# leggedrobotics/art_planner

Hardware: AMD Instinct MI355X
Metric: validated states/sec on 400x400@0.04m map (sample + validity check) (higher is better)
Workload: dtype f32; 1 GPU; C2: lazy_prm_star_min_update front end, 400x400@0.04m Perlin terrain (seed 1234) + 12 obstacles, YAML robot, batch sampler + validity checker; map=400x400@0.04, lanes=1

## Files before the change

art_planner_amd/csrc/artp_capi.hip:

```cpp
#include "../../include/artp_c.h"

#include <hip/hip_runtime.h>
#include <hipcub/hipcub.hpp>

#include <cmath>
#include <cstdio>
#include <atomic>
#include <chrono>
#include <cstdlib>
#include <cstring>
#include <mutex>
#include <string>
#include <array>
#include <vector>

#include "pipeline.h"
#include "cost_kernels.h"

using namespace artp;

#define ARTP_FEW_STATES 16
#define ARTP_SVC_MAX_STATES 2
#define FEW_EDGE_S1 0
#define FEW_EDGE_S2 (ARTP_FEW_EDGES * 7 * sizeof(double))
// ... 12 lines not shown
  RobotDev robot{};
  MapGeom geom{};
  bool have_geom = false;
  std::atomic<uint64_t> map_version{0};
  FieldDev field[2]{};
  float* field_data[2] = {nullptr, nullptr};
  size_t field_elems[2] = {0, 0};
  bool have_field[2] = {false, false};
  void* rect_stage_host = nullptr;
  void* rect_stage_dev = nullptr;
  size_t rect_stage_cap = 0;
  hipEvent_t rect_stage_done = nullptr;
  hipEvent_t map_written = nullptr;
  hipEvent_t lane_mark[4] = {nullptr, nullptr, nullptr, nullptr};
  uint64_t map_write_seq = 0;
  uint64_t map_seen[4] = {0, 0, 0, 0};
  SamplerDev sampler{};
  float* sampler_buf = nullptr;
  float* sampler_pack = nullptr;
  int sampler_rows = 0, sampler_cols = 0;
  bool have_sampler = false;
  double z_low = 0.0, z_high = 0.0;
  bool have_z = false;
  int fc_mfma_wanted = 1;
  artp_cost_query_fn ext_cost_fn = nullptr;
  void* ext_cost_user = nullptr;
  bool few_edges = true;
  bool edge_two_pass = true;
  int edge_coarse_stride = ARTP_COARSE_STRIDE;
  float* table_buf[2] = {nullptr, nullptr};
  unsigned char* flag_buf[2] = {nullptr, nullptr};
  unsigned* stride_buf[2] = {nullptr, nullptr};
  unsigned char* partner_buf[2] = {nullptr, nullptr};
  unsigned* partner_cnt[2] = {nullptr, nullptr};
  int* d_diff = nullptr;
  int partner_R_built[2] = {-1, -1};
  int layer_has_nonfinite[2] = {1, 1};
  float4* tri_raw_buf[2] = {nullptr, nullptr};
  size_t table_elems[2] = {0, 0};
  TablesDev tables[2]{};
  ScratchCaps caps_full{0, 0, 0, 0};
  ScratchCaps caps_scan{0, 0, 0, 0};
  ScratchCaps caps_feet{0, 0, 0, 0};
  ScratchCaps caps_feet_wave{0, 0, 0, 0};
  ScratchCaps caps_foot_full{0, 0, 0, 0};
  int n_cus = 256;
  double* pin_states = nullptr;
  volatile uint8_t* pin_labels = nullptr;
  double* pin_states_dev = nullptr;
  uint8_t* pin_labels_dev = nullptr;
  bool poll_labels = true;
  bool svc_enabled = false, svc_launched = false;
  hipStream_t svc_stream = nullptr;
  hipEvent_t svc_after_map = nullptr;
  SvcMailbox* svc = nullptr;
  SvcMailbox* svc_dev = nullptr;
  uint32_t svc_seq = 0;
  uint64_t svc_map_version = 0;
  uint64_t svc_launches = 0, svc_requests = 0;
  bool pool_launched = false;
  hipStream_t pool_stream = nullptr;
  hipEvent_t pool_after_map = nullptr;
  EdgeMailbox* pool_mb = nullptr;
  int pool_bar = -1;
  PoolResponse* pool_resp = nullptr;
  PoolResponse* pool_resp_dev = nullptr;
  PoolCtl* pool_ctl = nullptr;
  uint64_t pool_shadow[5][7] = {};
  unsigned pool_wgs = ARTP_POOL_WGS;
  uint32_t pool_seq = 0;
  uint64_t pool_map_version = 0;
  uint64_t pool_launches = 0, pool_requests = 0;
  char* pin_edges_in = nullptr;
  char* pin_edges_in_dev = nullptr;
  char* pin_edges = nullptr;
  char* pin_edges_dev = nullptr;
  FewEdgeSync* d_few_sync = nullptr;
  int* d_error = nullptr;
  unsigned long long* d_count = nullptr;
  void* tmp[8] = {nullptr, nullptr, nullptr, nullptr, nullptr, nullptr, nullptr, nullptr};
  size_t tmp_cap[8] = {0, 0, 0, 0, 0, 0, 0, 0};
  void* cub_tmp = nullptr;
  size_t cub_cap = 0;
  struct lane_state {
    bool init = false;
    hipStream_t own_stream = nullptr, stream = nullptr;
    unsigned long long* d_count = nullptr;
    int* d_error = nullptr;
    void* tmp[8] = {nullptr, nullptr, nullptr, nullptr, nullptr, nullptr, nullptr, nullptr};
    size_t tmp_cap[8] = {0, 0, 0, 0, 0, 0, 0, 0};
    void* cub_tmp = nullptr;
    size_t cub_cap = 0;
  };
  lane_state lanes[ARTP_MAX_LANES];
  int cur_lane = 0;
  bool have_weights = false;
  int cost_net = 0;
  half8* d_convw[5] = {nullptr, nullptr, nullptr, nullptr, nullptr};
  float* d_convb[5] = {nullptr, nullptr, nullptr, nullptr, nullptr};
  float* d_c12 = nullptr;
  unsigned char* d_c12m = nullptr;
  int conv12_mfma = 1;
  half8* d_convw_chunk[3] = {nullptr, nullptr, nullptr};
  half8* d_convw_p32 = nullptr;
  float* d_fc = nullptr;
  char* d_fc_mfma = nullptr;
  int feet_dense = 0;
  double r3_extent_override = 0.0;
  int fc_mfma = 1;
  int fc_selfcheck = -1;
  float fc_selfcheck_err = 0.f;
  half_t* d_act[2] = {nullptr, nullptr};
  size_t act_cap = 0;
  half_t* d_feat = nullptr;
  size_t feat_cap = 0;
  float* d_map_f32 = nullptr;
  size_t map_cap = 0;
  CostMapGeom cost_geom{};
  int feat_h = 0, feat_w = 0;
  bool have_features = false;
  bool cost_fill_holes = false;
  bool cost_fill_telea = false;
  std::string last_error;
  std::string arch;
  std::recursive_mutex mu;
};

namespace {

#define HIP_TRY(ctx, expr)                                                        \
  do {                                                                            \
    hipError_t _e = (expr);                                                       \
    if (_e != hipSuccess) {                                                       \
      (ctx)->last_error = std::string(#expr) + ": " + hipGetErrorString(_e);      \
      return ARTP_ERR_HIP;                                                        \
    }                                                                             \
  } while (0)

int ensure_tmp(artp_ctx* c, int slot, size_t bytes) {
  if (c->tmp_cap[slot] >= bytes) return ARTP_OK;
  if (c->tmp[slot]) HIP_TRY(c, hipFree(c->tmp[slot]));
  c->tmp[slot] = nullptr;
  c->tmp_cap[slot] = 0;
  const size_t want = bytes + bytes / 4 + 256;
  HIP_TRY(c, hipMalloc(&c->tmp[slot], want));
  c->tmp_cap[slot] = want;
  return ARTP_OK;
}

void park_lane(artp_ctx* c) {
  artp_ctx::lane_state& l = c->lanes[c->cur_lane];
  l.init = true;
  l.own_stream = c->own_stream;
  l.stream = c->stream;
  l.d_count = c->d_count;
  l.d_error = c->d_error;
  l.cub_tmp = c->cub_tmp;
  l.cub_cap = c->cub_cap;
  for (int k = 0; k < 8; ++k) {
    l.tmp[k] = c->tmp[k];
    l.tmp_cap[k] = c->tmp_cap[k];
  }
}

void unpark_lane(artp_ctx* c, int lane) {
  const artp_ctx::lane_state& l = c->lanes[lane];
  c->own_stream = l.own_stream;
  c->stream = l.stream;
  c->d_count = l.d_count;
  c->d_error = l.d_error;
  c->cub_tmp = l.cub_tmp;
  c->cub_cap = l.cub_cap;
  for (int k = 0; k < 8; ++k) {
    c->tmp[k] = l.tmp[k];
    c->tmp_cap[k] = l.tmp_cap[k];
  }
  c->cur_lane = lane;
}

int order_after_other_lanes(artp_ctx* c) {
  for (int l = 0; l < ARTP_MAX_LANES; ++l) {
    if (l == c->cur_lane || !c->lanes[l].init) continue;
    if (!c->lane_mark[l]) HIP_TRY(c, hipEventCreateWithFlags(&c->lane_mark[l], hipEventDisableTiming));
    HIP_TRY(c, hipEventRecord(c->lane_mark[l], c->lanes[l].stream));
    HIP_TRY(c, hipStreamWaitEvent(c->stream, c->lane_mark[l], 0));
  }
  return ARTP_OK;
}

int publish_map_write(artp_ctx* c) {
  if (!c->map_written) HIP_TRY(c, hipEventCreateWithFlags(&c->map_written, hipEventDisableTiming));
  HIP_TRY(c, hipEventRecord(c->map_written, c->stream));
  c->map_seen[c->cur_lane] = ++c->map_write_seq;
  return ARTP_OK;
}

int lane_sees_map(artp_ctx* c) {
  if (c->map_seen[c->cur_lane] != c->map_write_seq && c->map_written) {
    HIP_TRY(c, hipStreamWaitEvent(c->stream, c->map_written, 0));
    c->map_seen[c->cur_lane] = c->map_write_seq;
  }
  return ARTP_OK;
}

void fill_robot(artp_ctx* c) {
  const artp_params& p = c->params;
  RobotDev& r = c->robot;
  r.torso[0] = (float)p.torso_length;
  r.torso[1] = (float)p.torso_width;
  r.torso[2] = (float)p.torso_height;
  r.foot[0] = (float)p.reach_x;
  r.foot[1] = (float)p.reach_y;
  r.foot[2] = (float)p.reach_z;
  r.torso_off[0] = (float)p.torso_off_x;
  r.torso_off[1] = (float)p.torso_off_y;
  r.torso_off[2] = (float)(p.torso_off_z - p.feet_off_z);
  r.feet_off_x = (float)p.feet_off_x;
  r.feet_off_y = (float)p.feet_off_y;
  r.unknown_space_untraversable = p.unknown_space_untraversable;
  r.reach_z = p.reach_z;
  r.max_pitch_pert = p.max_pitch_pert;
  r.max_roll_pert = p.max_roll_pert;
}

void r_from_2_axes(float* R, float ax, float ay, float az, float bx, float by, float bz) {
  float l = sqrtf(ax * ax + ay * ay + az * az);
  if (l <= 0.0f) return;
  l = 1.0f / l;
  ax *= l; ay *= l; az *= l;
  const float k = ax * bx + ay * by + az * bz;
  bx -= k * ax; by -= k * ay; bz -= k * az;
  l = sqrtf(bx * bx + by * by + bz * bz);
  if (l <= 0.0f) return;
  l = 1.0f / l;
  bx *= l; by *= l; bz *= l;
  R[0] = ax; R[4] = ay; R[8] = az;
  R[1] = bx; R[5] = by; R[9] = bz;
  R[2] = -by * az + ay * bz;
  R[6] = -bz * ax + az * bx;
  R[10] = -bx * ay + ax * by;
  R[3] = R[7] = R[11] = 0.0f;
}

int size_scratch(artp_ctx* c) {
  const artp_params& p = c->params;
  const double d_torso = std::sqrt(p.torso_length * p.torso_length + p.torso_width * p.torso_width +
                                   p.torso_height * p.torso_height);
  const double d_foot = std::sqrt(p.reach_x * p.reach_x + p.reach_y * p.reach_y + p.reach_z * p.reach_z);
  double diag = d_torso > d_foot ? d_torso : d_foot;
  double spacing = 1e30;
  int max_n = 2;
  for (int s = 0; s < 2; ++s) {
    if (!c->have_field[s]) continue;
    spacing = std::fmin(spacing, (double)std::fmin(c->field[s].sample_w, c->field[s].sample_d));
    max_n = std::max(max_n, std::max(c->field[s].nW, c->field[s].nD));
  }
  if (spacing > 1e29) return ARTP_OK;
  int maxdim = (int)std::ceil(diag / spacing) + 4;
  if (maxdim > max_n) maxdim = max_n;
  if (maxdim < 4) maxdim = 4;
  long verts = (long)maxdim * maxdim;
  long tris = 2L * (maxdim - 1) * (maxdim - 1);
  if (tris > 4096) tris = 4096;
  verts = (verts + 3) & ~3L;
  tris = (tris + 7) & ~7L;
  long tab = 64;
  while (tab < 2 * tris && tab < 4096) tab <<= 1;
  if (maxdim > 64) {
    c->last_error = "box window wider than 64 samples: not supported by the packed triangle ids";
    return ARTP_ERR_CAPACITY;
  }
  c->caps_full = ScratchCaps{64 * 36, (int)verts, (int)tris, (int)tab};
  c->caps_scan = ScratchCaps{64 * 36, (int)verts, (int)(tris < 1024 ? tris : 1024), 0};
  {
    int fdim = (int)std::ceil(d_foot / spacing) + 4;
    if (fdim > max_n) fdim = max_n;
    if (fdim < 4) fdim = 4;
    long fv = ((long)fdim * fdim + 3) & ~3L;
    long ft = (2L * (fdim - 1) * (fdim - 1) + 7) & ~7L;
    if (ft > 1024) ft = 1024;
    c->caps_feet = ScratchCaps{32 * 36, (int)fv, (int)ft, 0};
    c->caps_feet_wave = ScratchCaps{64 * 36, (int)fv, (int)ft, 0};
    long ftf = (2L * (fdim - 1) * (fdim - 1) + 7) & ~7L;
    if (ftf > 4096) ftf = 4096;
    long ftab = 64;
    while (ftab < 2 * ftf && ftab < 4096) ftab <<= 1;
    c->caps_foot_full = ScratchCaps{64 * 36, (int)fv, (int)ftf, (int)ftab};
  }
  if (scratch_bytes_per_wave(c->caps_full) > 160 * 1024 ||
      scratch_bytes_per_wave(c->caps_scan) * ARTP_WAVES_PER_BLOCK > 160 * 1024 ||
      scratch_bytes_per_wave(c->caps_full) + 4 * scratch_bytes_per_wave(c->caps_foot_full) > 160 * 1024) {
    c->last_error = "box too large for the LDS window tile";
    return ARTP_ERR_CAPACITY;
  }
  return ARTP_OK;
}

size_t lds_full(const artp_ctx* c) { return scratch_bytes_per_wave(c->caps_full); }
size_t lds_scan(const artp_ctx* c) { return scratch_bytes_per_wave(c->caps_scan) * ARTP_WAVES_PER_BLOCK; }
size_t lds_feet(const artp_ctx* c) { return scratch_bytes_per_wave(c->caps_feet) * 4 * ARTP_WAVES_PER_BLOCK; }
size_t lds_feet_wave(const artp_ctx* c) { return scratch_bytes_per_wave(c->caps_feet_wave) * ARTP_WAVES_PER_BLOCK; }
size_t lds_few(const artp_ctx* c) {
  return scratch_bytes_per_wave(c->caps_full) + 4 * scratch_bytes_per_wave(c->caps_foot_full);
}

int set_kernel_lds(artp_ctx* c) {
  HIP_TRY(c, hipFuncSetAttribute(reinterpret_cast<const void*>(check_boxes_kernel<1>),
                                 hipFuncAttributeMaxDynamicSharedMemorySize, (int)lds_full(c)));
  HIP_TRY(c, hipFuncSetAttribute(reinterpret_cast<const void*>(validate_states_kernel<1>),
                                 hipFuncAttributeMaxDynamicSharedMemorySize, (int)lds_full(c)));
  HIP_TRY(c, hipFuncSetAttribute(reinterpret_cast<const void*>(plane_stage_kernel<1>),
                                 hipFuncAttributeMaxDynamicSharedMemorySize, (int)lds_full(c)));
  HIP_TRY(c, hipFuncSetAttribute(reinterpret_cast<const void*>(validate_few_kernel),
                                 hipFuncAttributeMaxDynamicSharedMemorySize, (int)lds_few(c)));
  HIP_TRY(c, hipFuncSetAttribute(reinterpret_cast<const void*>(check_motions_few_kernel),
                                 hipFuncAttributeMaxDynamicSharedMemorySize, (int)lds_few(c)));
  HIP_TRY(c, hipFuncSetAttribute(reinterpret_cast<const void*>(resolve_boxes_kernel<ARTP_WAVES_PER_BLOCK, 64, 3>),
                                 hipFuncAttributeMaxDynamicSharedMemorySize, (int)lds_scan(c)));
  HIP_TRY(c, hipFuncSetAttribute(reinterpret_cast<const void*>(resolve_boxes_kernel<ARTP_WAVES_PER_BLOCK, 16, 1>),
                                 hipFuncAttributeMaxDynamicSharedMemorySize, (int)lds_feet(c)));
  HIP_TRY(c, hipFuncSetAttribute(reinterpret_cast<const void*>(resolve_boxes_kernel<ARTP_WAVES_PER_BLOCK, 64, 2>),
                                 hipFuncAttributeMaxDynamicSharedMemorySize, (int)lds_feet_wave(c)));
  return ARTP_OK;
}

int grid_full(const artp_ctx* c, size_t tasks) {
  size_t per_cu = (160 * 1024) / (lds_full(c) ? lds_full(c) : 1);
  if (per_cu > 16) per_cu = 16;
  if (per_cu < 1) per_cu = 1;
  size_t g = (size_t)c->n_cus * per_cu;
  if (tasks && tasks < g) g = tasks;
  return (int)(g ? g : 1);
}
int grid_scan(const artp_ctx* c, size_t lds) {
  size_t per_cu = (160 * 1024) / (lds ? lds : 1);
  if (per_cu > 8) per_cu = 8;
  if (per_cu < 1) per_cu = 1;
  return (int)((size_t)c->n_cus * per_cu);
}

unsigned grid_sub(const artp_ctx* c, int per_cu) {
  const unsigned g = (unsigned)c->n_cus * (unsigned)per_cu;
  return (g + ARTP_NSUB - 1) / ARTP_NSUB * ARTP_NSUB;
}

int partner_radius(const artp_ctx* c, int slot) {
  const FieldDev& f = c->field[slot];
  const float* side = slot == 1 ? c->robot.foot : c->robot.torso;
  const double diag = std::sqrt((double)side[0] * side[0] + (double)side[1] * side[1] + (double)side[2] * side[2]);
  const int R = (int)std::ceil(diag / std::fmin((double)f.sample_w, (double)f.sample_d)) + 3;
  return R > 63 ? -1 : R;
}

static void partner_rect_extent(const FieldDev& f, const PartnerRects& pr, int margin, int* max_cells, int* max_rows) {
  *max_cells = *max_rows = 1;
  for (int k = 0; k < pr.n; ++k) {
    const int nx = std::min(pr.x1[k] + margin, f.nW - 1) - std::max(pr.x0[k] - margin, 0) + 1;
    const int nz = std::min(pr.z1[k] + margin, f.nD - 1) - std::max(pr.z0[k] - margin, 0) + 1;
    *max_cells = std::max(*max_cells, nx * nz);
    *max_rows = std::max(*max_rows, pr.z1[k] - pr.z0[k] + 1);
  }
}

int build_partner_table_full(artp_ctx* c, int slot) {
  FieldDev& f = c->field[slot];
// ... 68 lines not shown
  FieldDev& f = c->field[slot];
  const int R = partner_radius(c, slot);
  int cells0, cellsR, rows;
  partner_rect_extent(f, pr, 0, &cells0, &rows);
  partner_rect_extent(f, pr, R, &cellsR, &rows);
  hipLaunchKernelGGL(tri_raw_rects_kernel, dim3((cells0 + 255) / 256, pr.n), dim3(256), 0, c->stream, f, pr,
                     c->tri_raw_buf[slot], c->partner_cnt[slot]);
  hipLaunchKernelGGL(partner_count_kernel<true>, dim3((cellsR + 255) / 256, rows, pr.n), dim3(256), 0, c->stream, f, R,
                     (const float4*)c->tri_raw_buf[slot], c->partner_cnt[slot], pr, 1);
  hipLaunchKernelGGL(partner_count_kernel<false>, dim3((cells0 + 255) / 256, 2 * R + 1, pr.n), dim3(256), 0, c->stream, f, R,
                     (const float4*)c->tri_raw_buf[slot], c->partner_cnt[slot], pr, 1);
  hipLaunchKernelGGL(partner_flags_from_counts_kernel, dim3((cellsR + 255) / 256, pr.n), dim3(256), 0, c->stream, f.nW, f.nD,
                     pr, R, (const unsigned*)c->partner_cnt[slot], c->partner_buf[slot]);
  HIP_TRY(c, hipGetLastError());
  c->partner_R_built[slot] = R;
  f.partner_flags = c->partner_buf[slot];
  f.partner_R = R;
  return ARTP_OK;
}

int build_tables(artp_ctx* c, int slot, const PartnerRects* pr = nullptr) {
  const FieldDev& f = c->field[slot];
  const size_t elems = (size_t)f.nW * f.nD;
  if (c->table_elems[slot] < elems) {
    if (c->table_buf[slot]) HIP_TRY(c, hipFree(c->table_buf[slot]));
    if (c->flag_buf[slot]) HIP_TRY(c, hipFree(c->flag_buf[slot]));
    if (c->stride_buf[slot]) HIP_TRY(c, hipFree(c->stride_buf[slot]));
    c->stride_buf[slot] = nullptr;
    if (c->partner_buf[slot]) HIP_TRY(c, hipFree(c->partner_buf[slot]));
    if (c->partner_cnt[slot]) HIP_TRY(c, hipFree(c->partner_cnt[slot]));
    c->partner_cnt[slot] = nullptr;
    HIP_TRY(c, hipMalloc(reinterpret_cast<void**>(&c->partner_cnt[slot]), elems * sizeof(unsigned)));
    if (c->tri_raw_buf[slot]) HIP_TRY(c, hipFree(c->tri_raw_buf[slot]));
    c->tri_raw_buf[slot] = nullptr;
    HIP_TRY(c, hipMalloc(reinterpret_cast<void**>(&c->tri_raw_buf[slot]), elems * sizeof(float4)));
    c->table_buf[slot] = nullptr;
    c->flag_buf[slot] = nullptr;
    c->partner_buf[slot] = nullptr;
    HIP_TRY(c, hipMalloc(reinterpret_cast<void**>(&c->partner_buf[slot]), (elems + 3) / 4 * 4));
    c->partner_R_built[slot] = -1;
    HIP_TRY(c, hipMalloc(reinterpret_cast<void**>(&c->table_buf[slot]), 12 * elems * sizeof(float)));
    HIP_TRY(c, hipMalloc(reinterpret_cast<void**>(&c->flag_buf[slot]), 6 * elems));
    HIP_TRY(c, hipMalloc(reinterpret_cast<void**>(&c->stride_buf[slot]), (elems / 2 + 3 * (f.nW + f.nD) + 16) * sizeof(unsigned)));
    c->table_elems[slot] = elems;
  }
  float2* mm[6];
  unsigned char* fl[6];
  for (int l = 0; l < 6; ++l) {
    mm[l] = reinterpret_cast<float2*>(c->table_buf[slot]) + (size_t)l * elems;
    fl[l] = reinterpret_cast<unsigned char*>(c->flag_buf[slot]) + (size_t)l * elems;
  }
  const int n = (int)elems;
  hipLaunchKernelGGL(table_level0_kernel, dim3((n + 255) / 256), dim3(256), 0, c->stream, f.data, n, mm[0], fl[0]);
  for (int l = 1; l < 6; ++l)
    hipLaunchKernelGGL(table_level_up_kernel, dim3((n + 255) / 256), dim3(256), 0, c->stream,
                       (const float2*)mm[l - 1], (const unsigned char*)fl[l - 1], f.nW, f.nD, 1 << (l - 1), mm[l],
                       fl[l]);
  HIP_TRY(c, hipGetLastError());
  TablesDev& t = c->tables[slot];
  t.mm = mm[2];
  t.fl = fl[2];
  t.stride = (unsigned)elems;
  t.has_nan = f.has_nan;
  t.has_nonfinite = c->layer_has_nonfinite[slot];
  {
    unsigned off[ARTP_STRIDE_LEVELS + 1] = {0};
    for (int l = 0; l < ARTP_STRIDE_LEVELS; ++l) {
      const int s = 2 << l;
      off[l + 1] = off[l] + (unsigned)(((f.nW + s - 1) / s) * ((f.nD + s - 1) / s));
    }
    t.st = c->stride_buf[slot];
    t.st_off1 = off[1];
    t.st_off2 = off[2];
    hipLaunchKernelGGL(stride_tables_kernel, dim3((off[3] + 255) / 256), dim3(256), 0, c->stream, t.mm, t.fl, t.stride,
                       f.nW, f.nD, off[1], off[2], off[3], c->stride_buf[slot]);
    HIP_TRY(c, hipGetLastError());
  }
  const int rc_partner = pr ? partner_update_end(c, slot, *pr) : build_partner_table_full(c, slot);
  if (rc_partner != ARTP_OK) return rc_partner;
  t.valid = 1;
  return ARTP_OK;
}

int ensure_recs(artp_ctx* c, size_t n) { return ensure_tmp(c, 7, n * sizeof(PoseRec)); }

int launch_validate_pipeline(artp_ctx* c, const double* se3, size_t n, uint8_t* valid, bool recs_ready = false) {
  if (n >= (1ull << 32)) {
    c->last_error = "batch too large (state index is 32 bit)";
    return ARTP_ERR_INVALID_ARG;
  }
  int rc = ensure_recs(c, n);
  if (rc) return rc;
  PoseRec* recs = static_cast<PoseRec*>(c->tmp[7]);
  if (!recs_ready)
    hipLaunchKernelGGL(pose_rec_kernel, dim3((unsigned)((n + 255) / 256)), dim3(256), 0, c->stream, c->field[0], se3, n,
                       recs);
  const size_t per_block_states = 64 * ARTP_CLASSIFY_SUB;
  const size_t n_blocks = (n + per_block_states - 1) / per_block_states;
  const size_t seg_t = ((n_blocks + ARTP_NSUB - 1) / ARTP_NSUB) * per_block_states;
  rc = ensure_tmp(c, 4, 5 * ARTP_NSUB * seg_t * sizeof(PendingBox));
  if (rc) return rc;
  const size_t ctr_bytes = 128 + (size_t)2 * ARTP_NSUB * 128;
  rc = ensure_tmp(c, 5, ctr_bytes + ((5 + 4 + 4) * n + 5 * (size_t)ARTP_NSUB * seg_t) * sizeof(unsigned) + 64);
  if (rc) return rc;
  PipelineQueues q;
  q.q1 = static_cast<PendingBox*>(c->tmp[4]);
  q.counters = static_cast<unsigned long long*>(c->tmp[5]);
  q.sub = q.counters + 16;
  q.seg_t = seg_t;
  q.q2 = reinterpret_cast<unsigned*>(static_cast<char*>(c->tmp[5]) + ctr_bytes);
  q.q3 = q.q2 + 5 * n;
  q.q5 = q.q3 + 4 * n;
  q.q4 = q.q5 + 4 * n;
  q.q6 = q.q4 + 4 * (size_t)ARTP_NSUB * seg_t;
  q.feet_base = (unsigned long long)ARTP_NSUB * seg_t;
  HIP_TRY(c, hipMemsetAsync(q.counters, 0, ctr_bytes, c->stream));
  const size_t per_block = 64 * ARTP_CLASSIFY_SUB;
  hipLaunchKernelGGL(classify_states_kernel, dim3((unsigned)((n + per_block - 1) / per_block)),
                     dim3(ARTP_CLASSIFY_THREADS), 0, c->stream,
                     c->field[0], c->field[1], c->tables[0], c->tables[1], c->geom, c->robot, (const PoseRec*)recs, n,
                     valid, q);
#ifdef ARTP_VARIANTS
  if (c->feet_dense)
    hipLaunchKernelGGL(feet_stream2_kernel<ARTP_STREAM_WAVES>, dim3(grid_sub(c, ARTP_FEET_WAVES_PER_SIMD)), dim3(64 * ARTP_STREAM_WAVES), 0,
                       c->stream, c->field[1], c->robot, q, valid);
  else
#endif
    hipLaunchKernelGGL(feet_stream_kernel<ARTP_STREAM_WAVES>, dim3(grid_sub(c, ARTP_FEET_WAVES_PER_SIMD)), dim3(64 * ARTP_STREAM_WAVES), 0,
                       c->stream, c->field[1], c->robot, q, valid);
  hipLaunchKernelGGL(feet_lane_kernel, dim3((unsigned)c->n_cus * 8), dim3(ARTP_LANE_THREADS), 0, c->stream,
                     c->field[1], c->robot, q, valid);
  {
    const ScratchCaps caps_stream{0, 0, 0, 0};
    const size_t lds_stream = 0;
    hipLaunchKernelGGL((resolve_boxes_kernel<ARTP_WAVES_PER_BLOCK, 64, 0>), dim3(grid_sub(c, ARTP_TORSO_WGS_PER_CU)),
                       dim3(64 * ARTP_WAVES_PER_BLOCK), lds_stream, c->stream, c->field[0], c->robot, q, valid,
                       caps_stream, c->d_error, c->tables[0].valid ? c->tables[0].mm : (const float2*)nullptr);
  }
  hipLaunchKernelGGL((resolve_boxes_kernel<ARTP_WAVES_PER_BLOCK, 64, 3>), dim3(grid_scan(c, lds_scan(c))),
                     dim3(64 * ARTP_WAVES_PER_BLOCK), lds_scan(c), c->stream, c->field[0], c->robot, q, valid,
                     c->caps_scan, c->d_error);
  hipLaunchKernelGGL((resolve_boxes_kernel<ARTP_WAVES_PER_BLOCK, 16, 1>), dim3(grid_scan(c, lds_feet(c))),
                     dim3(64 * ARTP_WAVES_PER_BLOCK), lds_feet(c), c->stream, c->field[1], c->robot, q, valid,
                     c->caps_feet, c->d_error);
  hipLaunchKernelGGL((resolve_boxes_kernel<ARTP_WAVES_PER_BLOCK, 64, 2>), dim3(grid_scan(c, lds_feet_wave(c))),
                     dim3(64 * ARTP_WAVES_PER_BLOCK), lds_feet_wave(c), c->stream, c->field[1], c->robot, q, valid,
                     c->caps_feet_wave, c->d_error);
  hipLaunchKernelGGL(plane_stage_kernel<1>, dim3(grid_full(c, 0)), dim3(64), lds_full(c), c->stream,
                     c->field[0], c->field[1], c->robot, q, valid, c->caps_full, c->d_error);
  HIP_TRY(c, hipGetLastError());
  return ARTP_OK;
}

int check_error_flag(artp_ctx* c) {
  int flag = 0;
  HIP_TRY(c, hipMemcpyAsync(&flag, c->d_error, sizeof(int), hipMemcpyDeviceToHost, c->stream));
  HIP_TRY(c, hipStreamSynchronize(c->stream));
  if (flag) {
    HIP_TRY(c, hipMemsetAsync(c->d_error, 0, sizeof(int), c->stream));
    c->last_error = "a box window exceeded the LDS tile capacity";
    return ARTP_ERR_CAPACITY;
  }
  return ARTP_OK;
}

}

extern "C" {

void artp_params_defaults(artp_params* p) {
  p->torso_length = 1.05; p->torso_width = 0.55; p->torso_height = 0.2;
  p->torso_off_x = 0.0; p->torso_off_y = 0.0; p->torso_off_z = 0.0;
  p->feet_off_x = 0.362; p->feet_off_y = 0.225; p->feet_off_z = -0.525;
  p->reach_x = 0.25; p->reach_y = 0.1; p->reach_z = 0.15;
  p->unknown_space_untraversable = 1;
  p->max_pitch_pert = 10.0 / 180 * M_PI;
  p->max_roll_pert = 3.33 / 180 * M_PI;
  p->sample_from_distribution = 1;
}

void artp_params_yaml(artp_params* p) {
  p->torso_length = 1.31; p->torso_width = 0.65; p->torso_height = 0.3;
  p->torso_off_x = 0.0; p->torso_off_y = 0.0; p->torso_off_z = 0.04;
  p->feet_off_x = 0.51; p->feet_off_y = 0.2; p->feet_off_z = -0.475;
  p->reach_x = 0.2; p->reach_y = 0.2; p->reach_z = 0.2;
  p->unknown_space_untraversable = 1;
  p->max_pitch_pert = 10 * M_PI / 180;
  p->max_roll_pert = 3.33 * M_PI / 180;
  p->sample_from_distribution = 1;
}

const char* artp_status_string(int s) {
  switch (s) {
    case ARTP_OK: return "ok";
    case ARTP_ERR_INVALID_ARG: return "invalid argument";
    case ARTP_ERR_NO_DEVICE: return "no usable HIP device (this library has no CPU fallback)";
    case ARTP_ERR_HIP: return "HIP runtime error";
    case ARTP_ERR_NO_MAP: return "required layer not uploaded";
    case ARTP_ERR_CAPACITY: return "box window exceeds the LDS tile capacity";
    case ARTP_ERR_NO_WEIGHTS: return "motion-cost weights not loaded";
    case ARTP_ERR_TIMEOUT: return "timed out waiting for a device group";
    case ARTP_ERR_COMM: return "RCCL unavailable or a communicator call failed";
    case ARTP_ERR_COST_FUNC: return "Motion cost call failed";
    default: return "unknown status";
  }
}

const char* artp_last_error(const artp_ctx* ctx) { return ctx ? ctx->last_error.c_str() : ""; }
const char* artp_device_arch(const artp_ctx* ctx) { return ctx ? ctx->arch.c_str() : ""; }

static void pool_stop(artp_ctx* c);
static void svc_stop(artp_ctx* c) {
  if (!c->svc || !c->svc_launched) return;
  c->svc->n_quit = 0x100u;
  std::atomic_thread_fence(std::memory_order_seq_cst);
  const auto t0 = std::chrono::steady_clock::now();
  while (c->svc->running && std::chrono::steady_clock::now() - t0 < std::chrono::milliseconds(200))
    ;
  (void)hipStreamSynchronize(c->svc_stream);
  c->svc_launched = false;
}

static int svc_start(artp_ctx* c) {
  if (!c->svc) {
    void *p = nullptr, *pd = nullptr;
    HIP_TRY(c, hipHostMalloc(&p, sizeof(SvcMailbox), hipHostMallocMapped));
    HIP_TRY(c, hipHostGetDevicePointer(&pd, p, 0));
    std::memset(p, 0, sizeof(SvcMailbox));
    c->svc = static_cast<SvcMailbox*>(p);
    c->svc_dev = static_cast<SvcMailbox*>(pd);
    HIP_TRY(c, hipStreamCreateWithFlags(&c->svc_stream, hipStreamNonBlocking));
    HIP_TRY(c, hipEventCreateWithFlags(&c->svc_after_map, hipEventDisableTiming));
    HIP_TRY(c, hipFuncSetAttribute(reinterpret_cast<const void*>(validate_service_kernel),
// ... 1435 lines not shown
  if (!c || (n && (!s1 || !s2 || !valid))) return ARTP_ERR_INVALID_ARG;
  if (n == 0) return ARTP_OK;
  std::lock_guard<std::recursive_mutex> lock(c->mu);
  HIP_TRY(c, hipSetDevice(c->device));
  double few_max = 0.0;
  if (n <= ARTP_FEW_EDGES && c->few_edges && c->have_field[0] && c->have_field[1] && (mode != 0 || c->have_z) &&
      few_edges_task_estimate(c, mode, s1, s2, n, &few_max) <= 65536.0) {
    if (c->svc_enabled && n <= ARTP_POOL_MAX_EDGES && few_max * n <= 8.0 * c->pool_wgs && pool_available(c))
      return run_edges_pool(c, mode, s1, s2, n, valid, aux_out, last_t, last_state);
    return run_edges_few(c, mode, true, s1, s2, n, valid, aux_out, last_t, last_state, few_max);
  }
  int rc = ensure_tmp(c, 0, 2 * n * 7 * sizeof(double));
  if (rc) return rc;
  rc = ensure_tmp(c, 1, n * 8 * sizeof(double) + n * 4 + n + 16);
  if (rc) return rc;
  HIP_TRY(c, hipMemcpyAsync(c->tmp[0], s1, n * 7 * sizeof(double), hipMemcpyHostToDevice, c->stream));
  HIP_TRY(c, hipMemcpyAsync(static_cast<double*>(c->tmp[0]) + 7 * n, s2, n * 7 * sizeof(double),
                            hipMemcpyHostToDevice, c->stream));
  double* d_last_t = static_cast<double*>(c->tmp[1]);
  double* d_last_state = d_last_t + n;
  uint32_t* d_aux = reinterpret_cast<uint32_t*>(d_last_state + 7 * n);
  uint8_t* d_valid = reinterpret_cast<uint8_t*>(d_aux + n);
  rc = run_edges_dev(c, mode, static_cast<const double*>(c->tmp[0]),
                     static_cast<const double*>(c->tmp[0]) + 7 * n, n, d_valid, d_aux,
                     last_t ? d_last_t : nullptr, last_state ? d_last_state : nullptr);
  if (rc) return rc;
  HIP_TRY(c, hipMemcpyAsync(valid, d_valid, n, hipMemcpyDeviceToHost, c->stream));
  if (aux_out) HIP_TRY(c, hipMemcpyAsync(aux_out, d_aux, n * sizeof(uint32_t), hipMemcpyDeviceToHost, c->stream));
  if (last_t) HIP_TRY(c, hipMemcpyAsync(last_t, d_last_t, n * sizeof(double), hipMemcpyDeviceToHost, c->stream));
  if (last_t && last_state)
    HIP_TRY(c, hipMemcpyAsync(last_state, d_last_state, n * 7 * sizeof(double), hipMemcpyDeviceToHost, c->stream));
  return check_error_flag(c);
}

int artp_set_edge_passes(artp_ctx* c, int two_pass, int coarse_stride) {
  if (!c || (coarse_stride != 0 && coarse_stride < 2)) return ARTP_ERR_INVALID_ARG;
  std::lock_guard<std::recursive_mutex> lock(c->mu);
  c->edge_two_pass = two_pass != 0;
  c->edge_coarse_stride = coarse_stride ? coarse_stride : ARTP_COARSE_STRIDE;
  return ARTP_OK;
}
int artp_set_few_edges(artp_ctx* c, int enabled) {
  if (!c) return ARTP_ERR_INVALID_ARG;
  std::lock_guard<std::recursive_mutex> lock(c->mu);
  c->few_edges = enabled != 0;
  return ARTP_OK;
}
int artp_check_motions_dev(artp_ctx* c, const double* s1, const double* s2, size_t n, uint8_t* valid) {
  return run_edges_dev(c, 0, s1, s2, n, valid, nullptr);
}
int artp_check_motions(artp_ctx* c, const double* s1, const double* s2, size_t n, uint8_t* valid) {
  return run_edges_host(c, 0, s1, s2, n, valid, nullptr);
}
int artp_check_motions_last_valid_dev(artp_ctx* c, const double* s1, const double* s2, size_t n, uint8_t* valid,
                                      double* last_valid_t, double* last_valid_se3) {
  if (n && !last_valid_t) return ARTP_ERR_INVALID_ARG;
  return run_edges_dev(c, 0, s1, s2, n, valid, nullptr, last_valid_t, last_valid_se3);
}
int artp_check_motions_last_valid(artp_ctx* c, const double* s1, const double* s2, size_t n, uint8_t* valid,
                                  double* last_valid_t, double* last_valid_se3) {
  if (n && !last_valid_t) return ARTP_ERR_INVALID_ARG;
  return run_edges_host(c, 0, s1, s2, n, valid, nullptr, last_valid_t, last_valid_se3);
}
int artp_check_edges_interp_dev(artp_ctx* c, const double* s1, const double* s2, size_t n,
                                uint8_t* valid, uint32_t* n_interp_out) {
  return run_edges_dev(c, 1, s1, s2, n, valid, n_interp_out);
}
int artp_check_edges_interp(artp_ctx* c, const double* s1, const double* s2, size_t n, uint8_t* valid,
                            uint32_t* n_interp_out) {
  return run_edges_host(c, 1, s1, s2, n, valid, n_interp_out);
}


namespace {
struct Se3Row { double v[7]; };
}

int artp_debug_pipeline_counters(artp_ctx* c, uint64_t out[8]) {
  if (!c || !out) return ARTP_ERR_INVALID_ARG;
  std::lock_guard<std::recursive_mutex> lock(c->mu);
  if (!c->tmp[5]) return ARTP_ERR_NO_MAP;
  HIP_TRY(c, hipSetDevice(c->device));
  uint64_t raw[16 + 2 * ARTP_NSUB * 16];
  HIP_TRY(c, hipMemcpyAsync(raw, c->tmp[5], sizeof(raw), hipMemcpyDeviceToHost, c->stream));
  HIP_TRY(c, hipStreamSynchronize(c->stream));
  for (int k = 0; k < 8; ++k) out[k] = raw[k];
  out[0] = out[4] = out[2] = out[7] = 0;
  for (int s = 0; s < ARTP_NSUB; ++s) {
    out[0] += raw[16 + (size_t)s * 16];
    out[4] += raw[16 + (size_t)(ARTP_NSUB + s) * 16];
    out[2] += raw[16 + (size_t)s * 16 + 2];
    out[7] += raw[16 + (size_t)(ARTP_NSUB + s) * 16 + 2];
  }
  return ARTP_OK;
}

int artp_debug_partner_table(artp_ctx* c, int slot, uint8_t* out, size_t out_bytes, int* radius) {
  if (!c || slot < 0 || slot > 1 || !radius) return ARTP_ERR_INVALID_ARG;
  std::lock_guard<std::recursive_mutex> lock(c->mu);
  if (!c->have_field[slot]) return ARTP_ERR_NO_MAP;
  const FieldDev& f = c->field[slot];
  *radius = f.partner_flags ? f.partner_R : 0;
  if (!out || !f.partner_flags) return ARTP_OK;
  const size_t need = (size_t)f.nW * f.nD;
  if (out_bytes < need) return ARTP_ERR_INVALID_ARG;
  HIP_TRY(c, hipSetDevice(c->device));
  HIP_TRY(c, hipMemcpyAsync(out, f.partner_flags, need, hipMemcpyDeviceToHost, c->stream));
  HIP_TRY(c, hipStreamSynchronize(c->stream));
  return ARTP_OK;
}

int artp_compact_valid_dev(artp_ctx* c, const double* se3, const uint8_t* valid, size_t n,
                           double* out_se3, uint64_t* n_out_dev) {
  if (!c || (n && (!se3 || !valid || !out_se3)) || !n_out_dev) return ARTP_ERR_INVALID_ARG;
  std::lock_guard<std::recursive_mutex> lock(c->mu);
  HIP_TRY(c, hipSetDevice(c->device));
  if (n == 0) {
    HIP_TRY(c, hipMemsetAsync(n_out_dev, 0, sizeof(uint64_t), c->stream));
    return ARTP_OK;
  }
  const Se3Row* in = reinterpret_cast<const Se3Row*>(se3);
  Se3Row* out = reinterpret_cast<Se3Row*>(out_se3);
  unsigned long long* cnt = reinterpret_cast<unsigned long long*>(n_out_dev);
  size_t need = 0;
  HIP_TRY(c, hipcub::DeviceSelect::Flagged(nullptr, need, in, valid, out, cnt, (int)n, c->stream));
  if (c->cub_cap < need) {
    if (c->cub_tmp) HIP_TRY(c, hipFree(c->cub_tmp));
    c->cub_tmp = nullptr;
    HIP_TRY(c, hipMalloc(&c->cub_tmp, need + 256));
    c->cub_cap = need + 256;
  }
  size_t cap = c->cub_cap;
  HIP_TRY(c, hipcub::DeviceSelect::Flagged(c->cub_tmp, cap, in, valid, out, cnt, (int)n, c->stream));
  return ARTP_OK;
}

int artp_compact_valid_indices_dev(artp_ctx* c, const uint8_t* valid, size_t n, uint32_t* out_idx,
                                   uint64_t* n_out_dev) {
  if (!c || (n && (!valid || !out_idx)) || !n_out_dev || n >= (1ull << 32)) return ARTP_ERR_INVALID_ARG;
  std::lock_guard<std::recursive_mutex> lock(c->mu);
  HIP_TRY(c, hipSetDevice(c->device));
  if (n == 0) {
    HIP_TRY(c, hipMemsetAsync(n_out_dev, 0, sizeof(uint64_t), c->stream));
    return ARTP_OK;
  }
  hipcub::CountingInputIterator<uint32_t> in(0u);
  unsigned long long* cnt = reinterpret_cast<unsigned long long*>(n_out_dev);
  size_t need = 0;
  HIP_TRY(c, hipcub::DeviceSelect::Flagged(nullptr, need, in, valid, out_idx, cnt, (int)n, c->stream));
  if (c->cub_cap < need) {
    if (c->cub_tmp) HIP_TRY(c, hipFree(c->cub_tmp));
    c->cub_tmp = nullptr;
    HIP_TRY(c, hipMalloc(&c->cub_tmp, need + 256));
    c->cub_cap = need + 256;
  }
  size_t cap = c->cub_cap;
  HIP_TRY(c, hipcub::DeviceSelect::Flagged(c->cub_tmp, cap, in, valid, out_idx, cnt, (int)n, c->stream));
  return ARTP_OK;
}

namespace {
__global__ void __launch_bounds__(256)
gather_edge_records_kernel(const uint32_t* __restrict__ sel, const unsigned long long* __restrict__ count,
                           const uint32_t* __restrict__ edge_i, const uint32_t* __restrict__ edge_j,
                           const float* __restrict__ cost, uint32_t* __restrict__ out) {
  const size_t n = (size_t)(*count);
  for (size_t e = (size_t)blockIdx.x * blockDim.x + threadIdx.x; e < n; e += (size_t)gridDim.x * blockDim.x) {
// ... 1140 lines not shown
```

art_planner_amd/csrc/pipeline.h:

```cpp
#pragma once

#include <hip/hip_fp16.h>

#include "kernels.h"

namespace artp {

#define ARTP_TABLE_LEVELS 4

struct TablesDev {
  const float2* mm;
  const unsigned char* fl;
  unsigned stride;
  int has_nan;
  int has_nonfinite;
  int valid;
  const unsigned* st;
  unsigned st_off1, st_off2;
};

#define ARTP_STRIDE_LEVELS 3

__global__ void __launch_bounds__(256)
table_level0_kernel(const float* __restrict__ data, int n, float2* __restrict__ mm, unsigned char* __restrict__ fl) {
// ... 635 lines not shown
    if (list_t)
      code2 = classify_tail(fb, tb, bb, true, rec.pad[1] != 0u, all_finite);
    else
      code2 = classify_tail(ff, tf, bb, false, rec.pad[1] != 0u, all_finite);
#endif
    codes[(origin >> 6) % SUB][(origin >> 6) / SUB][origin & 63] = (uint8_t)code2;
  }
  ARTP_C_MARK(5);
  __syncthreads();
  {
    bool pending = have && code2 >= 2;
    if (pending) {
      const int os = (origin >> 6) % SUB, ol = origin & 63;
#pragma unroll
      for (int kk = 0; kk < 5; ++kk) pending = pending && (codes[os][kk][ol] != 1);
    }
    const unsigned long long pbal = __ballot(pending);
    const int pc = __popcll(pbal);
    if (pc) {
      if (pending) {
        open_recs[6 * slot + 5] = make_float4(__uint_as_float(state), __uint_as_float(record_kind(list_t, code2 == 2, all_finite)), 0.0f, 0.0f);
        plist[wave * 64 + __popcll(pbal & lt_mask)] = (unsigned short)slot;
      }
      unsigned long long base = 0;
      if (lane == 0) {
        const int sq = blockIdx.x % ARTP_NSUB;
        base = sub_base(q, list_t ? 0 : 1, sq) + atomicAdd(sub_counter(q, list_t ? 0 : 1, sq), (unsigned long long)pc);
      }
      base = __shfl(base, 0);
      if (!list_t) {
        const bool nostat = pending && code2 == 3;
        const unsigned long long nbal = __ballot(nostat);
        if (nbal) {
          const int sq = blockIdx.x % ARTP_NSUB;
          unsigned long long fb = 0;
          if (lane == 0) fb = atomicAdd(sub_fwd(q, 1, sq), (unsigned long long)__popcll(nbal));
          fb = __shfl(fb, 0);
          if (nostat)
            q.q4[fwd_base(q, 1, sq) + fb + (unsigned long long)__popcll(nbal & lt_mask)] =
                (unsigned)(base + (unsigned long long)__popcll(pbal & lt_mask));
        }
      }
      wave_lds_sync();
      float4* out = reinterpret_cast<float4*>(q.q1 + base);
      const unsigned short* pl = plist + wave * 64;
      for (int j = lane; j < pc * 6; j += 64) {
        const int e = j / 6;
        out[j] = open_recs[6 * (int)pl[e] + (j - 6 * e)];
      }
    }
  }
  if (body && live) {
    bool ok = true;
#pragma unroll
    for (int kk = 0; kk < 5; ++kk) ok = ok && (codes[sub][kk][lane] != 1);
    valid[i] = (uint8_t)ok;
  }
  ARTP_C_MARK(6);
  ARTP_C_FLUSH(0);
}

#define ARTP_LANE_THREADS 256
#ifndef ARTP_LANE_SCAN_MIN
#define ARTP_LANE_SCAN_MIN 65536ull
#endif
#define ARTP_STREAM_WAVES 4
#ifndef ARTP_TORSO_WGS_PER_CU
#define ARTP_TORSO_WGS_PER_CU 14
#endif
#ifndef ARTP_TORSO_U
#define ARTP_TORSO_U 2
#endif
#ifndef ARTP_FEET_U
#define ARTP_FEET_U 4
#endif
#ifndef ARTP_FEET_CHUNK
#define ARTP_FEET_CHUNK 32
#endif
#ifndef ARTP_TORSO_CHUNK
#define ARTP_TORSO_CHUNK 8
#endif

__global__ void __launch_bounds__(ARTP_LANE_THREADS)
feet_lane_kernel(FieldDev ff, RobotDev rb, PipelineQueues q, uint8_t* __restrict__ valid) {
  const int tid = threadIdx.x;
  const int lane = tid & 63;
  const unsigned long long lt_mask = (lane == 0) ? 0ull : (~0ull >> (64 - lane));
  const unsigned long long count = fwd_total(q, 1);
  if (count < ARTP_LANE_SCAN_MIN) return;
  const unsigned long long stride = (unsigned long long)gridDim.x * blockDim.x;
  const unsigned long long rounds = (count + stride - 1) / stride;
  for (unsigned long long rnd = 0; rnd < rounds; ++rnd) {
    const unsigned long long it = rnd * stride + (unsigned long long)blockIdx.x * blockDim.x + tid;
    const bool live = it < count;
    const unsigned long long item = live ? (unsigned long long)fwd_item(q, 1, q.q4, it) : q.feet_base;
    bool undecided = false;
    if (live) {
      const PendingBox rec = q.q1[item];
      if (valid[rec.state] != 0) {
        BoxHF b;
        box_from_record(rec, rb, b);
        const int numX = b.maxX - b.minX + 1, numZ = b.maxZ - b.minZ + 1;
        const int cellsX = numX - 1, cellsZ = numZ - 1;
        const float minO2 = b.aabb[2];
        const int nW = ff.nW;
        const float* base = ff.data + b.minX + (size_t)b.minZ * nW;
        WindowStats w;
        w.maxY = -INFINITY;
        w.minY = INFINITY;
        w.allFinite = true;
        bool vhit = false;
        for (int xl = 0; xl < numX; ++xl) {
          const float vx = (float)(b.minX + xl) * ff.sample_w;
          for (int zl0 = 0; zl0 < numZ; zl0 += 8) {
           float hh[8];
#pragma unroll
           for (int k = 0; k < 8; ++k) hh[k] = (zl0 + k < numZ) ? base[xl + (zl0 + k) * nW] : 0.0f;
#pragma unroll
           for (int k = 0; k < 8; ++k) {
            const int zl = zl0 + k;
            if (zl >= numZ) break;
            const float* c = base + xl + zl * nW;
            const float h = hh[k];
            w.maxY = (w.maxY > h) ? w.maxY : h;
            if (is_finite(h)) {
              w.minY = (w.minY > h) ? h : w.minY;
              if (!vhit && h > minO2) {
                const float vz = (float)(b.minZ + zl) * ff.sample_d;
                if (point_in_box(b, vx, h, vz)) {
                  const bool xm = xl > 0, xp = xl < cellsX, zm = zl > 0, zp = zl < cellsZ;
                  const bool f_xp = xp && is_finite(c[1]);
                  const bool f_xm = xm && is_finite(c[-1]);
                  const bool f_zp = zp && is_finite(c[nW]);
                  const bool f_zm = zm && is_finite(c[-nW]);
                  const bool f_xm_zp = xm && zp && is_finite(c[nW - 1]);
                  const bool f_xp_zm = xp && zm && is_finite(c[1 - nW]);
                  vhit = (f_xp && f_zp) || (f_xm && f_xm_zp) || (f_xm_zp && f_zp) || (f_zm && f_xp_zm) ||
                         (f_xp_zm && f_xp) || (f_zm && f_xm);
                }
              }
            } else {
              w.allFinite = false;
            }
           }
          }
        }
        int result = 0, ec;
        bool decided = !(rec.kind & ARTP_REC_EXITS_NEGATIVE) && decide_exits(b, w, result, ec);
        if (!decided && vhit) {
          result = 1;
          decided = true;
        }
        if (decided && result == 0) valid[rec.state] = 0;
        undecided = !decided;
      }
    }
    const unsigned long long b3 = __ballot(undecided);
    unsigned long long base3 = 0;
    if (lane == 0 && b3) base3 = atomicAdd(&q.counters[5], (unsigned long long)__popcll(b3));
    base3 = __shfl(base3, 0, 64);
    if (undecided) q.q3[base3 + __popcll(b3 & lt_mask)] = (unsigned)item;
  }
}

#ifdef ARTP_STAGE_TIMING
__device__ unsigned long long g_feet_cycles[4];
#endif
#ifndef ARTP_FEET_WAVES_PER_SIMD
// ... 114 lines not shown
    const unsigned long long it = next;
    next += PASS == 0 ? 1ull : stride;
    const unsigned long long item =
        PASS == 0 ? first + it
                  : (unsigned long long)(PASS == 1 ? (direct ? fwd_item(q, 1, q.q4, it) : q.q3[it])
                                                   : (PASS == 2 ? q.q5[it] : fwd_item(q, 0, q.q6, it)));
#ifdef ARTP_STAGE_TIMING
    long long t_prev = clock64();
#endif
    const PendingBox rec = q.q1[item];
    if (valid[rec.state] == 0) continue;
    BoxHF b;
    box_from_record(rec, rb, b);
    ARTP_T_MARK(0);
    int result = 0, ec, fast_r = 2;
    bool decided = false;
    if constexpr (PASS == 0) {
      if (fld.partner_flags != nullptr && (rec.kind & ARTP_REC_ALL_FINITE)) {
        __shared__ unsigned short hot_blocks[WAVES][ARTP_HOT_BLOCKS];
        if (wave_vertex_stream_blocks<ARTP_TORSO_U>(fld, mm4, b, hot_blocks[threadIdx.x >> 6], lane)) {
          result = 1;
          decided = true;
        } else {
          ARTP_T_MARK(2);
          const int r = grp_corner_stage_direct<G>(fld, b, lane);
          if (r != 2) {
            result = r;
            decided = true;
          }
        }
        ARTP_T_MARK(4);
      }
      if (!decided) {
        if (gl == 0) fs[it - chunk_first] = (unsigned)item + 1u;
      } else if (gl == 0 && result != 0) {
        valid[rec.state] = 0;
      }
      continue;
    }
    const int total = (b.maxX - b.minX + 1) * (b.maxZ - b.minZ + 1);
    if (total > s.cap_verts) {
      if (gl == 0) atomicExch(error_flag, 1);
      continue;
    }
    WindowStats w;
    if (!decided) {
      grp_scan_window<G>(fld, b, s, lane, w);
      ARTP_T_MARK(1);
      decided = !feet && decide_exits(b, w, result, ec);
    }
    if (!decided) {
      const bool vhit = !feet && grp_vertex_pass<G>(fld, b, s, lane, w.allFinite);
      ARTP_T_MARK(2);
      if (vhit) {
        result = 1;
        decided = true;
      } else if (PASS == 1) {
        const int r = grp_plane_stage_corners<G>(fld, b, s, lane, 0, true);
        ARTP_T_MARK(4);
        if (r != 2) {
          result = r;
          decided = true;
        } else if (gl == 0) {
          const unsigned long long slot = atomicAdd(&q.counters[6], 1ull);
          q.q5[slot] = (unsigned)item;
        }
      } else if (PASS == 3 && fld.partner_flags != nullptr &&
                 (fast_r = grp_plane_stage_corners<G>(fld, b, s, lane, 0, true)) != 2) {
        ARTP_T_MARK(4);
        result = fast_r;
        decided = true;
      } else {
        const int T = grp_compact_triangles<G, true>(b, s, lane);
        ARTP_T_MARK(3);
#ifdef ARTP_STAGE_TIMING
        const int r = (T == 0) ? 0 : (T < 0 ? 2 : grp_plane_stage_corners<G>(fld, b, s, lane, T, false, t_acc));
#else
        const int r = (T == 0) ? 0 : (T < 0 ? 2 : grp_plane_stage_corners<G>(fld, b, s, lane, T));
#endif
        ARTP_T_MARK(4);
        if (r != 2) {
          result = r;
          decided = true;
        } else if (gl == 0) {
          const unsigned long long slot = atomicAdd(&q.counters[1], 1ull);
          q.q2[slot] = (unsigned)item;
        }
      }
    }
    if (decided && gl == 0) {
      const bool ok = (rec.kind & 1u) ? (result != 0) : (result == 0);
      if (!ok) valid[rec.state] = 0;
    }
    wave_lds_sync();
  }
#ifdef ARTP_STAGE_TIMING
  if (gl == 0) {
    for (int k = 0; k < 8; ++k) atomicAdd(&g_stage_cycles[G == 64 ? 0 : 1][k], t_acc[k]);
    atomicAdd(&g_stage_cycles[G == 64 ? 0 : 1][8], (unsigned long long)(clock64() - t_begin));
    atomicAdd(&g_stage_cycles[G == 64 ? 0 : 1][9], 1ull);
  }
#endif
}

template <int WAVES>
__global__ void __launch_bounds__(64 * WAVES)
plane_stage_kernel(FieldDev fb, FieldDev ff, RobotDev rb, PipelineQueues q, uint8_t* __restrict__ valid,
                   ScratchCaps caps, int* __restrict__ error_flag) {
  extern __shared__ __attribute__((aligned(16))) char smem[];
  const int lane = threadIdx.x & 63;
  const WaveScratch s = carve_scratch(smem, threadIdx.x >> 6, caps);
  const unsigned long long count = q.counters[1];
  const unsigned long long stride = (unsigned long long)gridDim.x * WAVES;
  for (unsigned long long item = (unsigned long long)blockIdx.x * WAVES + (threadIdx.x >> 6); item < count;
       item += stride) {
    const PendingBox rec = q.q1[q.q2[item]];
    if (valid[rec.state] == 0) continue;
    BoxHF b;
    box_from_record(rec, rb, b);
    const bool foot = (rec.kind & 1u) != 0;
    WindowStats w;
    if (foot)
      wave_scan_window(ff, b, s, lane, w);
    else
      wave_scan_window(fb, b, s, lane, w);
    const int T = wave_compact_triangles<true>(b, s, lane);
    if (T < 0) {
      if (lane == 0) atomicExch(error_flag, 1);
      continue;
    }
    const int result = (T > 0 && (foot ? wave_plane_stage(ff, b, s, lane, T) : wave_plane_stage(fb, b, s, lane, T))) ? 1 : 0;
    if (lane == 0) {
      const bool ok = (rec.kind & 1u) ? (result != 0) : (result == 0);
      if (!ok) valid[rec.state] = 0;
    }
    wave_lds_sync();
  }
}

#ifdef ARTP_VARIANTS
#include "pipeline_variants.h"
#endif

}
```

Baseline: 3.678 billion states/s.

## Double-buffer pipeline counters cleared in-kernel and resolve feet boxes in-wave

The per-call memset of the pipeline counters is replaced by two parity-alternating counter blocks. The feet_lane kernel zeroes the block for the next call, so a separate memset launch is no longer needed each batch. It also gives the per-wave feet scratch a hash table, so pass-2 boxes that the corner test leaves undecided run the full plane stage in place instead of being queued for a later kernel. This trades an extra stage and queue hand-off for longer per-wave work and larger LDS use. It adds error-path cleanup of the counter buffer and reads stats from the previous parity.

```diff
diff --git a/art_planner_amd/csrc/artp_capi.hip b/art_planner_amd/csrc/artp_capi.hip
--- a/art_planner_amd/csrc/artp_capi.hip
+++ b/art_planner_amd/csrc/artp_capi.hip
@@ -118,6 +118,7 @@
   size_t tmp_cap[8] = {0, 0, 0, 0, 0, 0, 0, 0};
   void* cub_tmp = nullptr;
   size_t cub_cap = 0;
+  int ctr_parity = 0;
   struct lane_state {
     bool init = false;
     hipStream_t own_stream = nullptr, stream = nullptr;
@@ -127,6 +128,7 @@
     size_t tmp_cap[8] = {0, 0, 0, 0, 0, 0, 0, 0};
     void* cub_tmp = nullptr;
     size_t cub_cap = 0;
+    int ctr_parity = 0;
   };
   lane_state lanes[ARTP_MAX_LANES];
   int cur_lane = 0;
@@ -193,6 +195,7 @@
   l.d_error = c->d_error;
   l.cub_tmp = c->cub_tmp;
   l.cub_cap = c->cub_cap;
+  l.ctr_parity = c->ctr_parity;
   for (int k = 0; k < 8; ++k) {
     l.tmp[k] = c->tmp[k];
     l.tmp_cap[k] = c->tmp_cap[k];
@@ -207,6 +210,7 @@
   c->d_error = l.d_error;
   c->cub_tmp = l.cub_tmp;
   c->cub_cap = l.cub_cap;
+  c->ctr_parity = l.ctr_parity;
   for (int k = 0; k < 8; ++k) {
     c->tmp[k] = l.tmp[k];
     c->tmp_cap[k] = l.tmp_cap[k];
@@ -316,7 +320,9 @@
     long ft = (2L * (fdim - 1) * (fdim - 1) + 7) & ~7L;
     if (ft > 1024) ft = 1024;
     c->caps_feet = ScratchCaps{32 * 36, (int)fv, (int)ft, 0};
-    c->caps_feet_wave = ScratchCaps{64 * 36, (int)fv, (int)ft, 0};
+    long fwtab = 64;
+    while (fwtab < 2 * ft && fwtab < 4096) fwtab <<= 1;
+    c->caps_feet_wave = ScratchCaps{64 * 36, (int)fv, (int)ft, (int)fwtab};
     long ftf = (2L * (fdim - 1) * (fdim - 1) + 7) & ~7L;
     if (ftf > 4096) ftf = 4096;
     long ftab = 64;
@@ -551,6 +557,8 @@
   return ARTP_OK;
 }
 
+constexpr size_t kPipelineCtrBytes = 128 + (size_t)2 * ARTP_NSUB * 128;
+
 int ensure_recs(artp_ctx* c, size_t n) { return ensure_tmp(c, 7, n * sizeof(PoseRec)); }
 
 int launch_validate_pipeline(artp_ctx* c, const double* se3, size_t n, uint8_t* valid, bool recs_ready = false) {
@@ -569,21 +577,24 @@
   const size_t seg_t = ((n_blocks + ARTP_NSUB - 1) / ARTP_NSUB) * per_block_states;
   rc = ensure_tmp(c, 4, 5 * ARTP_NSUB * seg_t * sizeof(PendingBox));
   if (rc) return rc;
-  const size_t ctr_bytes = 128 + (size_t)2 * ARTP_NSUB * 128;
-  rc = ensure_tmp(c, 5, ctr_bytes + ((5 + 4 + 4) * n + 5 * (size_t)ARTP_NSUB * seg_t) * sizeof(unsigned) + 64);
+  const size_t ctr_bytes = kPipelineCtrBytes;
+  const size_t cap5 = c->tmp_cap[5];
+  rc = ensure_tmp(c, 5, 2 * ctr_bytes + ((5 + 4 + 4) * n + 5 * (size_t)ARTP_NSUB * seg_t) * sizeof(unsigned) + 64);
   if (rc) return rc;
   PipelineQueues q;
   q.q1 = static_cast<PendingBox*>(c->tmp[4]);
-  q.counters = static_cast<unsigned long long*>(c->tmp[5]);
+  q.counters = reinterpret_cast<unsigned long long*>(static_cast<char*>(c->tmp[5]) + c->ctr_parity * ctr_bytes);
+  unsigned long long* ctr_next =
+      reinterpret_cast<unsigned long long*>(static_cast<char*>(c->tmp[5]) + (c->ctr_parity ^ 1) * ctr_bytes);
   q.sub = q.counters + 16;
   q.seg_t = seg_t;
-  q.q2 = reinterpret_cast<unsigned*>(static_cast<char*>(c->tmp[5]) + ctr_bytes);
+  q.q2 = reinterpret_cast<unsigned*>(static_cast<char*>(c->tmp[5]) + 2 * ctr_bytes);
   q.q3 = q.q2 + 5 * n;
   q.q5 = q.q3 + 4 * n;
   q.q4 = q.q5 + 4 * n;
   q.q6 = q.q4 + 4 * (size_t)ARTP_NSUB * seg_t;
   q.feet_base = (unsigned long long)ARTP_NSUB * seg_t;
-  HIP_TRY(c, hipMemsetAsync(q.counters, 0, ctr_bytes, c->stream));
+  if (c->tmp_cap[5] != cap5) HIP_TRY(c, hipMemsetAsync(c->tmp[5], 0, 2 * ctr_bytes, c->stream));
   const size_t per_block = 64 * ARTP_CLASSIFY_SUB;
   hipLaunchKernelGGL(classify_states_kernel, dim3((unsigned)((n + per_block - 1) / per_block)),
                      dim3(ARTP_CLASSIFY_THREADS), 0, c->stream,
@@ -598,7 +609,7 @@
     hipLaunchKernelGGL(feet_stream_kernel<ARTP_STREAM_WAVES>, dim3(grid_sub(c, ARTP_FEET_WAVES_PER_SIMD)), dim3(64 * ARTP_STREAM_WAVES), 0,
                        c->stream, c->field[1], c->robot, q, valid);
   hipLaunchKernelGGL(feet_lane_kernel, dim3((unsigned)c->n_cus * 8), dim3(ARTP_LANE_THREADS), 0, c->stream,
-                     c->field[1], c->robot, q, valid);
+                     c->field[1], c->robot, q, valid, ctr_next, (unsigned)(ctr_bytes / sizeof(unsigned long long)));
   {
     const ScratchCaps caps_stream{0, 0, 0, 0};
     const size_t lds_stream = 0;
@@ -617,7 +628,15 @@
                      c->caps_feet_wave, c->d_error);
   hipLaunchKernelGGL(plane_stage_kernel<1>, dim3(grid_full(c, 0)), dim3(64), lds_full(c), c->stream,
                      c->field[0], c->field[1], c->robot, q, valid, c->caps_full, c->d_error);
-  HIP_TRY(c, hipGetLastError());
+  const hipError_t launch_rc = hipGetLastError();
+  if (launch_rc != hipSuccess) {
+    (void)hipStreamSynchronize(c->stream);
+    (void)hipFree(c->tmp[5]);
+    c->tmp[5] = nullptr;
+    c->tmp_cap[5] = 0;
+    HIP_TRY(c, launch_rc);
+  }
+  c->ctr_parity ^= 1;
   return ARTP_OK;
 }
 
@@ -2219,7 +2238,9 @@
   if (!c->tmp[5]) return ARTP_ERR_NO_MAP;
   HIP_TRY(c, hipSetDevice(c->device));
   uint64_t raw[16 + 2 * ARTP_NSUB * 16];
-  HIP_TRY(c, hipMemcpyAsync(raw, c->tmp[5], sizeof(raw), hipMemcpyDeviceToHost, c->stream));
+  static_assert(sizeof(raw) == kPipelineCtrBytes, "counter layout");
+  HIP_TRY(c, hipMemcpyAsync(raw, static_cast<const char*>(c->tmp[5]) + (c->ctr_parity ^ 1) * kPipelineCtrBytes,
+                            sizeof(raw), hipMemcpyDeviceToHost, c->stream));
   HIP_TRY(c, hipStreamSynchronize(c->stream));
   for (int k = 0; k < 8; ++k) out[k] = raw[k];
   out[0] = out[4] = out[2] = out[7] = 0;
diff --git a/art_planner_amd/csrc/pipeline.h b/art_planner_amd/csrc/pipeline.h
--- a/art_planner_amd/csrc/pipeline.h
+++ b/art_planner_amd/csrc/pipeline.h
@@ -741,8 +741,11 @@
 #endif
 
 __global__ void __launch_bounds__(ARTP_LANE_THREADS)
-feet_lane_kernel(FieldDev ff, RobotDev rb, PipelineQueues q, uint8_t* __restrict__ valid) {
+feet_lane_kernel(FieldDev ff, RobotDev rb, PipelineQueues q, uint8_t* __restrict__ valid,
+                 unsigned long long* __restrict__ ctr_next, unsigned n_ctr) {
   const int tid = threadIdx.x;
+  if (blockIdx.x == 0)
+    for (unsigned i = tid; i < n_ctr; i += ARTP_LANE_THREADS) ctr_next[i] = 0ull;
   const int lane = tid & 63;
   const unsigned long long lt_mask = (lane == 0) ? 0ull : (~0ull >> (64 - lane));
   const unsigned long long count = fwd_total(q, 1);
@@ -1023,6 +1026,10 @@
         if (r != 2) {
           result = r;
           decided = true;
+        } else if (PASS == 2 && T > 0 && s.tab_size >= 2 * T) {
+          wave_lds_sync();
+          result = wave_plane_stage(fld, b, s, lane, T) ? 1 : 0;
+          decided = true;
         } else if (gl == 0) {
           const unsigned long long slot = atomicAdd(&q.counters[1], 1ull);
           q.q2[slot] = (unsigned)item;
```

After: 3.697 billion states/s (median of 6 runs). Within noise of the previous version (+0.5%).
